# umutdundar99/progressive-stable-diffusion

Hardware: AMD Instinct MI355X
Metric: images/sec at 512x512, 50 DDIM steps, bs/GPU=4 (higher is better)
Workload: dtype f16; 1 GPU; 512x512, 50 DDIM steps, bs=4/GPU, delta-steer lambda=3.0, routing gates on, conditioning prep + VAE decode included; global_batch=4, parallelism=batch-shard x1 + 1 all-gather of uint8 frames

## Files before the change

### progressive-stable-diffusion_amd/csrc/bf16_names.h

```cpp
#pragma once
#define DADD_BF16 1

#define IgemmArgs IgemmArgs_bf16

#define igemm_kernel igemm_kernel_bf16
#define splitk_finish_kernel splitk_finish_kernel_bf16
#define splitk_finish_gn_kernel splitk_finish_gn_kernel_bf16
#define splitk_finish_gnapply_kernel splitk_finish_gnapply_kernel_bf16
#define igemm_dma_kernel igemm_dma_kernel_bf16
#define conv3x3_halo_kernel conv3x3_halo_kernel_bf16
#define gn_stats_kernel gn_stats_kernel_bf16
#define gn_apply_kernel gn_apply_kernel_bf16
#define gn_fused_kernel gn_fused_kernel_bf16
#define gn_reduce_kernel gn_reduce_kernel_bf16
#define layernorm_kernel layernorm_kernel_bf16
#define flash_kernel flash_kernel_bf16
#define xattn_kernel xattn_kernel_bf16
#define conv_in_nchw_kernel conv_in_nchw_kernel_bf16
#define conv_in_nchw_gn_kernel conv_in_nchw_gn_kernel_bf16
#define conv_cout4_kernel conv_cout4_kernel_bf16

#define dadd_init_igemm dadd_init_igemm_bf16
#define dadd_init_igemm_dma dadd_init_igemm_dma_bf16
#define dadd_launch_igemm_dma dadd_launch_igemm_dma_bf16
#define dadd_igemm_dma_persistent dadd_igemm_dma_persistent_bf16
#define dadd_init_conv_halo dadd_init_conv_halo_bf16
#define dadd_conv_halo_applicable dadd_conv_halo_applicable_bf16
#define dadd_conv_halo_gn_channels dadd_conv_halo_gn_channels_bf16
#define dadd_launch_conv_halo dadd_launch_conv_halo_bf16
#define dadd_init_norm dadd_init_norm_bf16
#define dadd_init_attention dadd_init_attention_bf16

#define dadd_conv_igemm_f16 dadd_conv_igemm_bf16
#define dadd_groupnorm_f16 dadd_groupnorm_bf16
#define dadd_layernorm_f16 dadd_layernorm_bf16
#define dadd_attn_f16 dadd_attn_bf16
#define dadd_attn_debug dadd_attn_debug_bf16
#define dadd_self_attn_f16 dadd_self_attn_bf16
#define dadd_tri_xattn_f16 dadd_tri_xattn_bf16
#define dadd_conv_in_nchw_f16 dadd_conv_in_nchw_bf16
#define dadd_conv3x3_cout4_f16 dadd_conv3x3_cout4_bf16
#define dadd_conv_out_ddim_f16 dadd_conv_out_ddim_bf16
```

### progressive-stable-diffusion_amd/csrc/igemm.hip

```cpp
#include "dadd_common.h"
#include "igemm_args.h"
#include <cstdlib>
#include <string>
#include "igemm_epilogue.h"

namespace {

constexpr int BM = 128;
constexpr int BK = 64;

__device__ __forceinline__ int lds_off(int row, int chunk) {
  return (row * 8 + (chunk ^ ((row >> 1) & 7))) * 8;
}

template <int BM, int BN, bool DEEP>
__global__ __launch_bounds__(256, 2) void igemm_kernel(const IgemmArgs p) {
  constexpr int WM = BM / 2;
  constexpr int MI = WM / 16;
  constexpr int WN = BN / 2;
  constexpr int J = WN / 16;
  constexpr int NA = BM * 8 / 256;
  constexpr int NB = BN * 8 / 256;
  extern __shared__ __attribute__((aligned(16))) char smem[];
  half_t* As = reinterpret_cast<half_t*>(smem);
// ... 512 lines not shown
  if (dma && tile_m == 128 && dadd_igemm_dma_persistent(a, nsplit) &&
      ((d->flags & DADD_TUNE_SHALLOW) ? false : 2.0 * a.B * a.Hi * a.Wi * Cin >= 2.0 * a.N * a.K))
    a.gm = a.gn = 0;
  const bool halo = dma && tile_m == 128 && dadd_conv_halo_applicable(a, tile_n);
  int halo_ns = 1;
  if (halo) {
    const int chunks = Cin / BK;
    int sk = d->splitk > 1 ? d->splitk : 1;
    if (sk > chunks) sk = chunks;
    a.kps = (chunks + sk - 1) / sk;
    halo_ns = (chunks + a.kps - 1) / a.kps;
    a.splitk = halo_ns;
    DADD_REQUIRE(halo_ns == 1 || a.partial != nullptr, "igemm: split-K needs a partial buffer");
  }
  if ((a.flags & DADD_EPI_GNSTAT) && (halo ? halo_ns : nsplit) > 1) {
    const int cb = (a.N % 160 == 0) ? 160 : 128, howo = a.Ho * a.Wo;
    const int rows = a.gn_nchunk > 0 ? howo / a.gn_nchunk : 0;
    DADD_REQUIRE(a.gn_ws && a.gn_cg > 0 && a.N == 32 * a.gn_cg && !geglu && a.counters == nullptr && a.N % cb == 0 &&
                     cb % a.gn_cg == 0 && (rows == 16 || rows == 64) && a.M % rows == 0 && howo % rows == 0 &&
                     a.gn_nchunk * rows == howo && !(a.flags & (DADD_EPI_LNFOLD | DADD_EPI_ACT_MASK)),
                 "igemm: GroupNorm statistics with split-K need the finish kernel (no tickets), N == 32 groups in blocks of "
                 "160 / 128 columns, and chunks of 16 or 64 rows: gn_nchunk == Ho*Wo / 16 (or / 64)");
  } else if (a.flags & DADD_EPI_GNSTAT) {
    const int wm_rows = tile_m / 2, wn_cols = tile_n / 2, howo = a.Ho * a.Wo;
    DADD_REQUIRE(a.gn_ws && a.gn_cg > 0 && a.N == 32 * a.gn_cg && !geglu && (tile_n == 128 || tile_n == 160) &&
                     wn_cols % a.gn_cg == 0 && a.M % tile_m == 0 && a.N % tile_n == 0 && howo % wm_rows == 0 &&
                     a.gn_nchunk == howo / wm_rows && !(a.flags & (DADD_EPI_LNFOLD | DADD_EPI_ACT_MASK)),
                 "igemm: GroupNorm statistics need full tiles of 128/160 columns holding whole groups, whole-wave row blocks "
                 "inside one sample (Ho*Wo %% %d == 0, gn_nchunk == Ho*Wo / %d), N == 32 groups, no split-K", wm_rows, wm_rows);
  }
  if (a.flags & DADD_EPI_GNAPPLY) {
    DADD_REQUIRE((halo ? halo_ns : nsplit) > 1 && a.counters == nullptr && a.gno_out && a.gno_gamma && a.gno_beta &&
                     a.gno_eps > 0.f && a.N % 64 == 0 && a.ldo % 2 == 0 && a.ldr % 2 == 0 &&
                     (size_t)a.Ho * a.Wo * (a.N / 32) * 2 <= 16 * 1024 && dadd_aligned16(a.gno_out) &&
                     !(a.flags & (DADD_EPI_GNSTAT | DADD_EPI_LNFOLD | DADD_EPI_LNSTAT | DADD_EPI_ACT_MASK)),
                 "igemm: GroupNorm of the output in the finish kernel needs a finish-kernel split-K launch, gn_out / gamma / "
                 "beta / eps, N %% 64 == 0, a (sample, group) slab of <= 16 KiB and no other statistics / activation flags");
  } else {
    DADD_REQUIRE(!(a.flags & DADD_EPI_GNAPPLY_SILU), "igemm: DADD_EPI_GNAPPLY_SILU without DADD_EPI_GNAPPLY");
  }
  if (a.flags & DADD_EPI_LNSTAT) {
    const int wn_cols = tile_n / 2;
    DADD_REQUIRE(a.ln_stats_out && !geglu && !halo && a.N % wn_cols == 0 && d->ln_parts_out == a.N / wn_cols &&
                     (nsplit == 1 || a.counters != nullptr) && !(a.flags & DADD_EPI_GNSTAT),
                 "igemm: LayerNorm row partials need ln_stats_out, N %% (tile_n/2) == 0, ln_parts_out == N / (tile_n/2) = %d, "
                 "no GEGLU and no finish-kernel split-K", a.N / wn_cols);
  }
  if (a.flags & DADD_PRE_GN) {
    const int cgc = Cin / 32;
    DADD_REQUIRE(a.C2 == 0 || (a.gni_ws2 && a.gni_nchunk2 >= 1 && a.gni_nchunk2 <= 256 && cgc > 0 && a.C1 % 32 == 0 &&
                               a.C2 % 32 == 0 && cgc % (a.C1 / 32) == 0 && cgc % (a.C2 / 32) == 0 && a.C1 % cgc == 0),
                 "igemm: GroupNorm over a concatenation needs the partials of both sources and group widths that nest "
                 "((C1+C2)/32 a multiple of C1/32 and C2/32, dividing C1)");
    DADD_REQUIRE(halo && !(d->flags & DADD_TUNE_SHALLOW) && Cin <= dadd_conv_halo_gn_channels(a.Wo) &&
                     Cin % 32 == 0 && a.gni_ws &&
                     a.gni_gamma && a.gni_beta && a.gni_nchunk >= 1 && a.gni_nchunk <= 256 && a.gni_eps > 0.f,
                 "igemm: GroupNorm on the way in needs the 3x3 halo kernel (stride 1, 64/32/16-wide map, 128x160 tiles), "
                 "Cin <= 1152 / 2048 / 2432 (W = 64 / 32 / 16), the chunk partials (<= 256 chunks), gamma, beta and eps");
  } else {
    DADD_REQUIRE(!(a.flags & DADD_PRE_GN_SILU), "igemm: DADD_PRE_GN_SILU without DADD_PRE_GN");
  }
  if (halo) {
    if (d->flags & DADD_TUNE_SHALLOW) a.flags |= DADD_TUNE_SHALLOW;
    rc = dadd_launch_conv_halo(a, halo_ns, s);
  }
  else if (dma)
    rc = dadd_launch_igemm_dma(a, tile_m, tile_n, nsplit, s);
  else if (tile_m == 128)
    rc = (tile_n == 160) ? launch<128, 160, false>(a, nsplit, s) : launch2<128, 128>(a, nsplit, deep, s);
  else
    rc = (tile_n == 160) ? launch2<64, 160>(a, nsplit, deep, s) : launch2<64, 128>(a, nsplit, deep, s);
  if (rc != DADD_OK) return rc;
  if ((halo ? halo_ns : nsplit) > 1 && a.counters == nullptr) {
    const size_t total = (size_t)a.M * (a.N / 4);
    int blocks = (int)((total + 255) / 256);
    if (blocks > 2048) blocks = 2048;
    const int ns = halo ? halo_ns : nsplit;
    const DaddLaunchTag tag = {(a.flags & DADD_EPI_GNSTAT) ? DADD_KNAME("splitk_finish_gn_kernel") : DADD_KNAME("splitk_finish_kernel"), 0.0,
                               (double)a.M * a.N * (4.0 * ns + 2.0 + ((a.flags & DADD_EPI_RESIDUAL) ? 2.0 : 0.0))};
    if (a.flags & DADD_EPI_GNAPPLY) {
      const DaddLaunchTag tag2 = {DADD_KNAME("splitk_finish_gnapply_kernel"), 0.0, tag.bytes + 2.0 * a.M * a.N};
      const unsigned slab_bytes = (unsigned)(a.Ho * a.Wo * (a.N / 32) * 2);
      if ((a.N / 32) % 4 == 0 && a.ldo % 4 == 0 && a.ldr % 4 == 0 && a.ld_rowvec % 4 == 0)
        dadd_launch(tag2, splitk_finish_gnapply_kernel<4>, dim3(32, a.B), dim3(512), slab_bytes, s, a, ns);
      else
        dadd_launch(tag2, splitk_finish_gnapply_kernel<2>, dim3(32, a.B), dim3(512), slab_bytes, s, a, ns);
    } else if (!(a.flags & DADD_EPI_GNSTAT))
      dadd_launch(tag, splitk_finish_kernel, dim3(blocks), dim3(256), 0, s, a, ns);
    else {
      const int rows = (a.Ho * a.Wo) / a.gn_nchunk;
      if (a.N % 160 == 0) {
        if (rows == 16) dadd_launch(tag, splitk_finish_gn_kernel<160, 16>, dim3(a.M / 16, a.N / 160), dim3(256), 0, s, a, ns);
        else dadd_launch(tag, splitk_finish_gn_kernel<160, 64>, dim3(a.M / 64, a.N / 160), dim3(256), 0, s, a, ns);
      } else {
        if (rows == 16) dadd_launch(tag, splitk_finish_gn_kernel<128, 16>, dim3(a.M / 16, a.N / 128), dim3(256), 0, s, a, ns);
        else dadd_launch(tag, splitk_finish_gn_kernel<128, 64>, dim3(a.M / 64, a.N / 128), dim3(256), 0, s, a, ns);
      }
    }
    DADD_LAUNCH_CHECK();
  }
  return DADD_OK;
}
```

### progressive-stable-diffusion_amd/csrc/igemm_args.h

```cpp
#pragma once
#include "dadd_common.h"

struct IgemmArgs {
  const half_t* x;
  const half_t* x2;
  const half_t* w;
  half_t* out;
  float* partial;
  const float* bias;
  const float* rowvec;
  const half_t* residual;
  int* counters;
  float* gn_ws;
  int gn_nchunk, gn_cg;
  const float* ln_c1;
  float ln_eps;
  float* ln_stats_out;
  const float* ln_stats_in;
  int ln_parts_in;
  const float* gni_ws;
  const float* gni_gamma;
  const float* gni_beta;
  int gni_nchunk;
  float gni_eps;
// ... 25 lines not shown
    const int per = p.gm * p.ntiles;
    const int g = tile_id / per, idx = tile_id - g * per;
    const int base = g * p.gm;
    const int gsz = min(p.gm, p.mtiles - base);
    mt = base + idx % gsz;
    nt = idx / gsz;
  } else if (p.gm >= p.mtiles) {
    const int per = p.mtiles * p.gn;
    const int g = tile_id / per, idx = tile_id - g * per;
    mt = idx % p.mtiles;
    nt = g * p.gn + idx / p.mtiles;
  } else {
    const int per = p.gm * p.gn;
    const int g = tile_id / per, idx = tile_id - g * per;
    const int ngn = p.ntiles / p.gn;
    const int gmi = g / ngn, gni = g - gmi * ngn;
    mt = gmi * p.gm + idx % p.gm;
    nt = gni * p.gn + idx / p.gm;
  }
}

static inline double dadd_igemm_flop(const IgemmArgs& a) { return 2.0 * (double)a.M * (double)a.N * (double)a.K; }
static inline double dadd_igemm_bytes(const IgemmArgs& a) {
  const double n_out = (a.flags & DADD_EPI_GEGLU) ? a.N / 2 : a.N;
  return 2.0 * ((double)a.B * a.Hi * a.Wi * (a.C1 + a.C2) + (double)a.N * a.K + (double)a.M * n_out +
                ((a.flags & DADD_EPI_RESIDUAL) ? (double)a.M * a.N : 0.0));
}

typedef half_t dadd_h2 __attribute__((ext_vector_type(2)));
__device__ __forceinline__ void ln_acc_pair(const h8& x, int p, float& s1, float& s2) {
  const dadd_h2 v = {x[2 * p], x[2 * p + 1]};
  const dadd_h2 one = {(half_t)1.0f, (half_t)1.0f};
  s1 = dadd_fdot2(v, one, s1);
  s2 = dadd_fdot2(v, v, s2);
}
template <int MI>
__device__ __forceinline__ void ln_finish(float (&s1)[MI], float (&s2)[MI], int K, float eps) {
  const float inv = 1.0f / (float)K;
#pragma unroll
  for (int i = 0; i < MI; ++i) {
    float a = s1[i], q = s2[i];
    a = dadd_sum_x16x32(a);
    q = dadd_sum_x16x32(q);
    const float mu = a * inv;
    const float var = fmaxf(q * inv - mu * mu, 0.f);
    s1[i] = mu;
    s2[i] = rsqrtf(var + eps);
  }
}

int dadd_init_igemm_dma();
int dadd_launch_igemm_dma(const IgemmArgs& a, int tile_m, int tile_n, int nsplit, hipStream_t s);
bool dadd_igemm_dma_persistent(const IgemmArgs& a, int nsplit);
int dadd_init_conv_halo();
bool dadd_conv_halo_applicable(const IgemmArgs& a, int tile_n);
int dadd_conv_halo_gn_channels(int Wo);
int dadd_launch_conv_halo(const IgemmArgs& a, int nsplit, hipStream_t s);
```

### progressive-stable-diffusion_amd/csrc/igemm_dma.hip

```cpp
#include "dadd_common.h"
#include "igemm_args.h"
#include <cstdlib>
#include "igemm_epilogue.h"

namespace {

constexpr int BK = 64;

typedef __attribute__((address_space(3))) void* lptr_t;
constexpr unsigned OOB = 0x80000000u;

__device__ __forceinline__ int lds_off(int row, int chunk) {
  return (row * 8 + (chunk ^ ((row >> 1) & 7))) * 8;
}

template <int N>
__device__ __forceinline__ void wait_vmcnt() {
  asm volatile("s_waitcnt vmcnt(%0)" ::"n"(N) : "memory");
}

template <int BM, int BN, bool UPS, bool PERS, int LNK>
__global__ __launch_bounds__(512, (BM + BN) <= 128 ? 4 : 2) void igemm_dma_kernel(const IgemmArgs p) {
#if defined(__HIP_DEVICE_COMPILE__)
  constexpr bool WS = true;
  constexpr bool LNF = LNK == 1;
  constexpr int WM = BM / 2, MI = WM / 16;
  constexpr int WN = BN / 2;
  constexpr int J = WN / 16;
  constexpr int NA = BM / 32;
  constexpr int NBJ = BN / 32;
  constexpr int LPT = NA + NBJ;
  constexpr int A_BYTES = BM * BK * 2, B_BYTES = BN * BK * 2, STAGE = A_BYTES + B_BYTES;
  extern __shared__ __attribute__((aligned(1024))) char smem[];

  const int t = threadIdx.x, lane = t & 63;
  const int wave_all = __builtin_amdgcn_readfirstlane(t >> 6);
  const bool loader = WS && wave_all >= 4;
  const int wave = WS ? (wave_all & 3) : wave_all;
  const int wm = wave >> 1, wn = wave & 1;
  int tile_first, tile_count;
  if constexpr (PERS) {
    const int total = p.mtiles * p.ntiles, nwg = gridDim.x;
    const int l = xcd_remap(blockIdx.x, nwg);
    const int q = total / nwg, r = total - q * nwg;
    tile_first = l * q + min(l, r);
    tile_count = q + (l < r ? 1 : 0);
  } else {
    tile_first = xcd_remap(blockIdx.x, gridDim.x);
    tile_count = 1;
  }
  const int z = PERS ? 0 : blockIdx.y;
  const int kt0 = PERS ? 0 : z * p.kps;
  const int kt1 = PERS ? p.nkt : min(p.nkt, kt0 + p.kps);
  const int nk = kt1 - kt0;
  const int Cin = p.C1 + p.C2;
  const int Hv = UPS ? 2 * p.Hi : p.Hi;
  const int Wv = UPS ? 2 * p.Wi : p.Wi;
  const int HoWo = p.Ho * p.Wo;
  const int lrow = lane >> 3, lch = lane & 7;

  const int shift1 = UPS ? 0 : (p.pad * p.Wi + p.pad) * p.C1;
  const int shift2 = UPS ? 0 : (p.pad * p.Wi + p.pad) * p.C2;
  const size_t pix_total = (size_t)p.B * p.Hi * p.Wi;
  const int rec1 = (int)((pix_total * p.C1 + shift1) * 2);
  const int rec2 = (int)((pix_total * p.C2 + shift2) * 2);
  const int recW = (int)((size_t)p.N * p.K * 2);
  const half_t* base1 = p.x - shift1;
  const half_t* base2 = (p.x2 ? p.x2 : p.x) - shift2;

  unsigned a_v1[NA], a_v2[NA], a_mask[NA];
  int a_pix[NA], a_y[NA], a_x[NA], a_cc[NA];
  unsigned w_v[NBJ];
  auto setup_tile = [&](int tile_id) {
  int nt, mt;
// ... 124 lines not shown
  const int total_kt = tile_count * nk;
  char* const ln_scr = smem + 4 * STAGE;
  const bool ln_stage = LNK == 2 && !UPS && ln_lds_usable(p, BM, nk);
  const bool ln_sts = ln_stage && ln_lds_stats(p, LN_LDS_BYTES);
  if (loader) {
    const int ln_extra = ln_stage ? ln_lds_count(p, wave, ln_sts) : 0;
    issue();
    issue();
    issue();
    wait_vmcnt<LPT>();
    __builtin_amdgcn_s_barrier();
    bool ext_young = false;
    int kc = 0, ext_tile = tile_first;
    for (int it = 0; it < total_kt; ++it) {
      if (it > 0) {
        if (ext_young) {
          switch (ln_extra) {
            case 1: wait_vmcnt<LPT + 1>(); break;
            case 2: wait_vmcnt<LPT + 2>(); break;
            case 3: wait_vmcnt<LPT + 3>(); break;
            case 4: wait_vmcnt<LPT + 4>(); break;
            default: wait_vmcnt<LPT>(); break;
          }
          ext_young = false;
        } else {
          wait_vmcnt<LPT>();
        }
        __builtin_amdgcn_s_barrier();
      }
      issue();
      if (ln_stage) {
        if (kc == 0) {
          int nt, mt;
          tile_decode(p, ext_tile, mt, nt);
          ln_lds_issue<BN>(p, ln_scr, __builtin_amdgcn_readfirstlane(mt) * BM, __builtin_amdgcn_readfirstlane(nt) * BN, wave,
                           lane, ln_sts);
          ext_young = ln_extra > 0;
          ++ext_tile;
        }
        kc = kc + 1 == nk ? 0 : kc + 1;
      }
    }
    wait_vmcnt<0>();
    return;
  }
  f4 acc[J][MI];
  const int fq = lane >> 4;
  int fa[2], fb[2];
#pragma unroll
  for (int s2 = 0; s2 < 2; ++s2) {
    fa[s2] = lds_off(wm * WM + (lane & 15), s2 * 4 + fq) * 2;
    fb[s2] = A_BYTES + lds_off(wn * WN + (lane & 15), s2 * 4 + fq) * 2;
  }
  __builtin_amdgcn_s_barrier();
  __builtin_amdgcn_sched_barrier(0);
  h8 xa0[MI], wb0[J], xa1[MI], wb1[J];
#pragma unroll
  for (int i = 0; i < MI; ++i) xa0[i] = *reinterpret_cast<const h8*>(smem + fa[0] + i * 2048);
#pragma unroll
  for (int j = 0; j < J; ++j) wb0[j] = *reinterpret_cast<const h8*>(smem + fb[0] + j * 2048);
  int comp_off = 0;
  bool started = false;
  for (int tl = 0; tl < tile_count; ++tl) {
#pragma unroll
    for (int j = 0; j < J; ++j)
#pragma unroll
      for (int i = 0; i < MI; ++i) acc[j][i] = f4{0.f, 0.f, 0.f, 0.f};
    [[maybe_unused]] float ls1[MI], ls2[MI];
    constexpr int LQ = MI * 4, LPER = (LQ + MI * J - 1) / (MI * J);
    if constexpr (LNF) {
#pragma unroll
      for (int i = 0; i < MI; ++i) ls1[i] = ls2[i] = 0.f;
    }
    for (int it = 0; it < nk; ++it) {
      if (started) __builtin_amdgcn_s_barrier();
      started = true;
      __builtin_amdgcn_sched_barrier(0);
      const int n1 = comp_off + STAGE;
      const int next_off = n1 >= 4 * STAGE ? 0 : n1;
      const char* ca = smem + comp_off + fa[1];
      const char* cb1 = smem + comp_off + fb[1];
      const char* na = smem + next_off + fa[0];
      const char* nb = smem + next_off + fb[0];
#pragma unroll
      for (int k = 0; k < MI * J; ++k) {
        const int jj = k / MI, ii = k % MI;
        acc[jj][ii] = DADD_MFMA_16X16X32(wb0[jj], xa0[ii], acc[jj][ii], 0, 0, 0);
        if constexpr (LNF) {
#pragma unroll
          for (int t2 = 0; t2 < LPER; ++t2)
            if (k * LPER + t2 < LQ) ln_acc_pair(xa0[(k * LPER + t2) / 4], (k * LPER + t2) % 4, ls1[(k * LPER + t2) / 4], ls2[(k * LPER + t2) / 4]);
        }
        if (k == 0) wb1[0] = *reinterpret_cast<const h8*>(cb1);
        else if (k <= MI) xa1[k - 1] = *reinterpret_cast<const h8*>(ca + (k - 1) * 2048);
        else if (k < MI + J) wb1[k - MI] = *reinterpret_cast<const h8*>(cb1 + (k - MI) * 2048);
        __builtin_amdgcn_sched_barrier(0);
      }
#pragma unroll
      for (int k = 0; k < MI * J; ++k) {
        const int jj = k / MI, ii = k % MI;
        acc[jj][ii] = DADD_MFMA_16X16X32(wb1[jj], xa1[ii], acc[jj][ii], 0, 0, 0);
        if constexpr (LNF) {
#pragma unroll
          for (int t2 = 0; t2 < LPER; ++t2)
            if (k * LPER + t2 < LQ) ln_acc_pair(xa1[(k * LPER + t2) / 4], (k * LPER + t2) % 4, ls1[(k * LPER + t2) / 4], ls2[(k * LPER + t2) / 4]);
        }
        if (k == 0) wb0[0] = *reinterpret_cast<const h8*>(nb);
        else if (k <= MI) xa0[k - 1] = *reinterpret_cast<const h8*>(na + (k - 1) * 2048);
        else if (k < MI + J) wb0[k - MI] = *reinterpret_cast<const h8*>(nb + (k - MI) * 2048);
        __builtin_amdgcn_sched_barrier(0);
      }
      comp_off = next_off;
      __builtin_amdgcn_sched_barrier(0);
    }
    int nt, mt;
    tile_decode(p, tile_first + tl, mt, nt);
    if constexpr (LNF) {
      ln_finish<MI>(ls1, ls2, p.K, p.ln_eps);
      igemm_epilogue<J, MI, WM, WN>(p, acc, mt * BM, nt * BN, wm, wn, lane, z, smem, ls1, ls2);
    } else {
      igemm_epilogue<J, MI, WM, WN>(p, acc, mt * BM, nt * BN, wm, wn, lane, z, smem, nullptr, nullptr, smem + 4 * STAGE,
                                    ln_sts ? ln_scr + LN_LDS_STATS : nullptr, ln_stage ? ln_scr : nullptr);
    }
  }
#endif
}

template <int BM, int BN>
constexpr int smem_bytes() {
  return 4 * (BM + BN) * BK * 2 + (BM == 128 ? LN_LDS_BYTES : 4096);
}

template <int BM, int BN, bool UPS, bool PERS, int LNK>
int set_attr() {
  DADD_HIP(hipFuncSetAttribute(reinterpret_cast<const void*>(&igemm_dma_kernel<BM, BN, UPS, PERS, LNK>),
                               hipFuncAttributeMaxDynamicSharedMemorySize, smem_bytes<BM, BN>()));
  return DADD_OK;
}

int g_num_cu = 0;

template <int BM, int BN, bool UPS, bool PERS, int LNK>
void launch1(const char* name, const IgemmArgs& a, dim3 grid, hipStream_t s) {
  dadd_launch({name, dadd_igemm_flop(a), dadd_igemm_bytes(a)}, igemm_dma_kernel<BM, BN, UPS, PERS, LNK>, grid, dim3(512),
              smem_bytes<BM, BN>(), s, a);
}
template <int BM, int BN, bool UPS, bool PERS>
void launch(const char* const (&names)[3], const IgemmArgs& a, dim3 grid, hipStream_t s) {
  if constexpr (!UPS) {
    if ((a.flags & DADD_EPI_LNFOLD) && a.ln_stats_in == nullptr) {
      launch1<BM, BN, false, PERS, 1>(names[1], a, grid, s);
      return;
    }
    if constexpr (BM == 128) {
      if (a.flags & DADD_EPI_LNFOLD) {
        launch1<BM, BN, false, PERS, 2>(names[2], a, grid, s);
        return;
      }
    }
  }
  launch1<BM, BN, UPS, PERS, 0>(names[0], a, grid, s);
}
template <int BM, int BN, bool PERS>
int set_attr2() {
  int rc = set_attr<BM, BN, false, PERS, 0>();
  if (rc == DADD_OK) rc = set_attr<BM, BN, false, PERS, 1>();
  if constexpr (BM == 128) {
    if (rc == DADD_OK) rc = set_attr<BM, BN, false, PERS, 2>();
  }
  return rc;
}

}

int dadd_init_igemm_dma() {
  int rc = set_attr2<128, 128, true>();
  if (rc == DADD_OK) rc = set_attr2<128, 160, true>();
  if (rc == DADD_OK) rc = set_attr2<128, 128, false>();
  if (rc == DADD_OK) rc = set_attr2<128, 160, false>();
  if (rc == DADD_OK) rc = set_attr<128, 128, true, false, 0>();
  if (rc == DADD_OK) rc = set_attr<128, 160, true, false, 0>();
  if (rc == DADD_OK) rc = set_attr2<64, 64, false>();
  if (rc == DADD_OK) rc = set_attr2<64, 128, false>();
  if (rc == DADD_OK) rc = set_attr2<64, 160, false>();
  int dev = 0;
  DADD_HIP(hipGetDevice(&dev));
  DADD_HIP(hipDeviceGetAttribute(&g_num_cu, hipDeviceAttributeMultiprocessorCount, dev));
  return rc;
}

bool dadd_igemm_dma_persistent(const IgemmArgs& a, int nsplit) {
  return (a.flags & DADD_TUNE_PERSIST) && nsplit == 1 && !a.ups && g_num_cu > 0 && a.mtiles * a.ntiles > g_num_cu;
}

int dadd_launch_igemm_dma(const IgemmArgs& a, int tile_m, int tile_n, int nsplit, hipStream_t s) {
  const int total = a.mtiles * a.ntiles;
  DADD_REQUIRE((size_t)a.B * a.Hi * a.Wi * (size_t)(a.C1 > a.C2 ? a.C1 : a.C2) * 2 < 0x7FF00000ull &&
                   (size_t)a.N * a.K * 2 < 0x7FF00000ull,
               "igemm(dma): operand larger than the 2 GiB buffer window");
  if (tile_m == 128 && dadd_igemm_dma_persistent(a, nsplit)) {
    dim3 grid(g_num_cu);
    if (tile_n == 160) { static const char* const nm[3] = {DADD_KNAME("igemm_dma_kernel") "<128, 160, false, true, 0>", DADD_KNAME("igemm_dma_kernel") "<128, 160, false, true, 1>", DADD_KNAME("igemm_dma_kernel") "<128, 160, false, true, 2>"}; launch<128, 160, false, true>(nm, a, grid, s); }
    else { static const char* const nm[3] = {DADD_KNAME("igemm_dma_kernel") "<128, 128, false, true, 0>", DADD_KNAME("igemm_dma_kernel") "<128, 128, false, true, 1>", DADD_KNAME("igemm_dma_kernel") "<128, 128, false, true, 2>"}; launch<128, 128, false, true>(nm, a, grid, s); }
    DADD_LAUNCH_CHECK();
    return DADD_OK;
  }
  dim3 grid(total, nsplit);
  if (tile_m == 64) {
    DADD_REQUIRE(!a.ups, "igemm(dma): the 64-row tiles have no upsample gather");
    if (tile_n == 160) { static const char* const nm[3] = {DADD_KNAME("igemm_dma_kernel") "<64, 160, false, false, 0>", DADD_KNAME("igemm_dma_kernel") "<64, 160, false, false, 1>", DADD_KNAME("igemm_dma_kernel") "<64, 160, false, false, 2>"}; launch<64, 160, false, false>(nm, a, grid, s); }
    else if (tile_n == 128) { static const char* const nm[3] = {DADD_KNAME("igemm_dma_kernel") "<64, 128, false, false, 0>", DADD_KNAME("igemm_dma_kernel") "<64, 128, false, false, 1>", DADD_KNAME("igemm_dma_kernel") "<64, 128, false, false, 2>"}; launch<64, 128, false, false>(nm, a, grid, s); }
    else { static const char* const nm[3] = {DADD_KNAME("igemm_dma_kernel") "<64, 64, false, false, 0>", DADD_KNAME("igemm_dma_kernel") "<64, 64, false, false, 1>", DADD_KNAME("igemm_dma_kernel") "<64, 64, false, false, 2>"}; launch<64, 64, false, false>(nm, a, grid, s); }
  } else if (tile_n == 160) {
    if (a.ups) { static const char* const nm[3] = {DADD_KNAME("igemm_dma_kernel") "<128, 160, true, false, 0>", DADD_KNAME("igemm_dma_kernel") "<128, 160, true, false, 1>", DADD_KNAME("igemm_dma_kernel") "<128, 160, true, false, 2>"}; launch<128, 160, true, false>(nm, a, grid, s); }
    else { static const char* const nm[3] = {DADD_KNAME("igemm_dma_kernel") "<128, 160, false, false, 0>", DADD_KNAME("igemm_dma_kernel") "<128, 160, false, false, 1>", DADD_KNAME("igemm_dma_kernel") "<128, 160, false, false, 2>"}; launch<128, 160, false, false>(nm, a, grid, s); }
  } else {
    if (a.ups) { static const char* const nm[3] = {DADD_KNAME("igemm_dma_kernel") "<128, 128, true, false, 0>", DADD_KNAME("igemm_dma_kernel") "<128, 128, true, false, 1>", DADD_KNAME("igemm_dma_kernel") "<128, 128, true, false, 2>"}; launch<128, 128, true, false>(nm, a, grid, s); }
    else { static const char* const nm[3] = {DADD_KNAME("igemm_dma_kernel") "<128, 128, false, false, 0>", DADD_KNAME("igemm_dma_kernel") "<128, 128, false, false, 1>", DADD_KNAME("igemm_dma_kernel") "<128, 128, false, false, 2>"}; launch<128, 128, false, false>(nm, a, grid, s); }
  }
  DADD_LAUNCH_CHECK();
  return DADD_OK;
}
```

### progressive-stable-diffusion_amd/engine.py

```python
from __future__ import annotations

import math
import os
from typing import Dict, List, Optional, Tuple

import torch

from . import lib as L
from .routing import get_block_type

F16, F32, BF16 = torch.float16, torch.float32, torch.bfloat16
OPERAND_DTYPES = (F16, BF16)
UNET_CH = (320, 640, 1280, 1280)
VAE_CH = (128, 256, 512, 512)
HEADS = 8
GROUPS = 32
N_CU = 256
FUSED_ATTN2 = os.environ.get("DADD_FUSED_ATTN2", "1") == "1"
A2_MIN_TILES = int(os.environ.get("DADD_A2_MIN_TILES", "128"))


def pack_conv(w: torch.Tensor, dtype=F16) -> torch.Tensor:
    if w.dim() == 2:
        return w.to(dtype).contiguous()
# ... 25 lines not shown

def fold_layernorm(w: torch.Tensor, b: Optional[torch.Tensor], gamma: torch.Tensor, beta: torch.Tensor, dtype=F16):
    w, gamma, beta = w.double(), gamma.double(), beta.double()
    w16 = (w * gamma[None, :]).to(dtype)
    bias = w @ beta + (b.double() if b is not None else 0.0)
    return w16, w16.double().sum(dim=1).float(), bias.float()


def lds_image(w: torch.Tensor) -> torch.Tensor:
    r = w.shape[0]
    sw = (torch.arange(r) >> 1) & 7
    idx = (torch.arange(8)[None, :] ^ sw[:, None])
    return w.reshape(r, 8, 8).gather(1, idx[:, :, None].expand(r, 8, 8)).reshape(r, 64).contiguous()


def pack_ffn_stream(w1: torch.Tensor, b1: torch.Tensor, w2: torch.Tensor, wp: torch.Tensor):
    c, hid = 320, 1280
    assert tuple(w1.shape) == (2 * hid, c) and tuple(w2.shape) == (c, hid) and tuple(wp.shape)[:2] == (c, c)
    w1, w2, wp = w1.to(F16), w2.to(F16), wp.reshape(c, c).to(F16)
    pieces, bias = [], []
    e = torch.arange(16)
    for ch in range(hid // 64):
        rows = []
        for wn in range(2):
            for u in range(2):
                h = ch * 64 + wn * 32 + u * 16 + e
                rows += [h, hid + h]
                bias += [b1[h].float(), b1[hid + h].float()]
        rows = torch.cat(rows)
        for kt in range(c // 64):
            pieces.append(lds_image(w1[rows][:, kt * 64:(kt + 1) * 64]))
        for nh in range(2):
            pieces.append(lds_image(w2[nh * 160:(nh + 1) * 160, ch * 64:(ch + 1) * 64]))
    for nh in range(2):
        for kt in range(c // 64):
            pieces.append(lds_image(wp[nh * 160:(nh + 1) * 160, kt * 64:(kt + 1) * 64]))
    return torch.cat([p.reshape(-1) for p in pieces]).contiguous(), torch.cat(bias).contiguous()


def pack_head_stream(wp: torch.Tensor, wq: torch.Tensor, wk: torch.Tensor, wv: torch.Tensor) -> torch.Tensor:
    c = 320
    wp = wp.reshape(c, c).to(F16)
    wqkv = torch.cat([wq, wk, wv]).to(F16)
    assert tuple(wqkv.shape) == (3 * c, c)
    pieces = []
    for w in (wp, wqkv):
        for nh in range(w.shape[0] // 160):
            for kt in range(c // 64):
                pieces.append(lds_image(w[nh * 160:(nh + 1) * 160, kt * 64:(kt + 1) * 64]))
    return torch.cat([p.reshape(-1) for p in pieces]).contiguous()


GN_IN_CONV = True

HALO_DUO = False

FINISH_GN_APPLY = True

WEIGHT_PREFETCH_AHEAD = int(os.environ.get("DADD_WEIGHT_PREFETCH", "0"))
WEIGHT_PREFETCH_MIN_BYTES = 2 * 1024 * 1024

GN_FROM_EPILOGUE = True
GN_FUSED_MAX_BYTES = 16 * 1024
SPLITK_GN_ROWS = 16


LN_FOLD = "auto"
LN_STATS_FROM_PRODUCER = True
LN_STATS_MAX_PARTS = 8


FUSED_FFN = True
FFN_MIN_BLOCKS = 128
FUSED_HEAD = True


def fold_here(m: int, n: int, k: int, geglu: bool = False) -> bool:
    if LN_FOLD == "auto":
        tile_m, _, _, tune = plan_tiling(m, n, k, 1, geglu, False)
        return tile_m == 64 and not (tune & L.TUNE_NODMA)
    return bool(LN_FOLD)


def choose_tiling(m: int, n: int, k: int, tile_n: int, geglu: bool = False,
                  residual: bool = True) -> Tuple[int, int, int]:
    nkt = k // 64
    nt = math.ceil(n / tile_n)
    t128 = math.ceil(m / 128) * nt
    if geglu:
        if m >= 16384:
            return 64, 1, L.TUNE_NODMA | L.TUNE_SHALLOW
        return 128, 1, (L.TUNE_PERSIST if t128 >= 4 * N_CU else 0)
    if nkt >= 12:
        if n <= 128 and nkt <= 18:
            return 128, 1, L.TUNE_NODMA
        per = 16 if t128 > 64 else (10 if t128 > 16 else 8)
        sk = max(1, min(round(N_CU / t128), nkt // per, 32))
        if not residual and nkt <= 20:
            sk = 1
        return 128, sk, (L.TUNE_PERSIST if sk == 1 and t128 >= 8 * N_CU else 0)
    if t128 > N_CU:
        return 128, 1, L.TUNE_PERSIST
    if not residual and nkt >= 5:
        return 128, 1, 0
    return (128 if t128 >= 2 * N_CU else 64), 1, L.TUNE_NODMA

# ... 133 lines not shown
                ws = self.be.zeros((out_shape[0] * (nchunk + extra) * GROUPS * 2,), F32)
                self.keep.append(ws)
                self.gn_partials[out.data_ptr()] = (ws, nchunk)
                gkw = dict(gn_ws=ws, gn_nchunk=nchunk)
                flags |= L.EPI_GNSTAT
        if (ln_stats and LN_STATS_FROM_PRODUCER and not (flags & (L.EPI_GEGLU | L.EPI_GNSTAT)) and sk == 1
                and n % (tile_n // 2) == 0 and n // (tile_n // 2) <= LN_STATS_MAX_PARTS):
            st = self.be.zeros((n // (tile_n // 2), m, 2), F32)
            self.keep.append(st)
            self.ln_partials[out.data_ptr()] = st
            gkw["ln_stats_out"] = st
            flags |= L.EPI_LNSTAT
        f = flags | (L.EPI_BIAS if bias is not None else 0) | (L.EPI_ROWVEC if rowvec is not None else 0) \
            | (L.EPI_RESIDUAL if residual is not None else 0) | (L.EPI_LNFOLD if ln_c1 is not None else 0) | tune
        kw = dict(ln_c1=ln_c1, ln_eps=ln_eps) if ln_c1 is not None else {}
        if (fuse_gn is not None and FINISH_GN_APPLY and sk > 1 and self.sk_counters is None and not (f & L.EPI_GNSTAT)
                and n % 64 == 0 and out_shape[1] * out_shape[2] * (n // 32) * 2 <= GN_FUSED_MAX_BYTES):
            g_out = self.pool.get(out_shape)
            f |= L.EPI_GNAPPLY | (L.EPI_GNAPPLY_SILU if fuse_gn[3] else 0)
            kw["gn_apply"] = (g_out, fuse_gn[0], fuse_gn[1], fuse_gn[2])
            self.gn_ready[out.data_ptr()] = (g_out, fuse_gn[0].data_ptr(), fuse_gn[1].data_ptr(), float(fuse_gn[2]), bool(fuse_gn[3]))
        if gn_in is not None:
            f |= L.PRE_GN | (L.PRE_GN_SILU if gn_in[5] else 0)
            kw["gn_in"] = tuple(gn_in[:5]) + tuple(gn_in[6:])
        if ln_c1 is not None and ln_stats_in is not None:
            kw["ln_stats_in"] = ln_stats_in
        self.rec(self.be.igemm, x, w, out, x2=x2, bias=bias, rowvec=rowvec, residual=residual,
                 taps=taps, stride=stride, ups=ups, pad=pad, flags=f, splitk=sk, partial=partial,
                 tile_n=tile_n, tile_m=tile_m, counters=self.sk_counters if sk > 1 else None, **kw, **gkw)
        self.pool.put(partial)
        return out

    def gn_in_conv_ok(self, x, x2, w, out_shape, residual) -> Optional[Tuple]:
        cmax = {64: 1152, 32: 2048, 16: 2432}.get(x.shape[2], 0)
        cin = x.shape[-1] + (0 if x2 is None else x2.shape[-1])
        if not GN_IN_CONV or cin > cmax or x.shape[-1] % 64 or cin % 64:
            return None
        part = self.gn_partials.get(x.data_ptr())
        if part is None or part[1] > 128:
            return None
        if x2 is not None:
            part2 = self.gn_partials.get(x2.data_ptr())
            c1_, c2_, cgc = x.shape[-1], x2.shape[-1], cin // 32
            if (part2 is None or part2[1] > 128 or c1_ % 32 or c2_ % 32 or cgc % (c1_ // 32) or cgc % (c2_ // 32)
                    or c1_ % cgc):
                return None
            part = (part[0], part[1], part2[0], part2[1])
        b, h, w_, _ = x.shape
        n, m = w.shape[0], out_shape[0] * out_shape[1] * out_shape[2]
        if tuple(out_shape[1:3]) != (h, w_) or h != w_ or w_ not in (16, 32, 64) or (h * w_) % 128:
            return None
        tile_m, tile_n, _, tune = plan_tiling(m, n, w.shape[1], 9, False, residual is not None, 0, 1)
        if tile_m != 128 or tile_n != 160 or (tune & (L.TUNE_NODMA | L.TUNE_PERSIST)) or HALO_DUO:
            return None
        return part

    def gn(self, x1, x2, gamma, beta, eps, silu):
        c = x1.shape[-1] + (0 if x2 is None else x2.shape[-1])
        ready = self.gn_ready.get(x1.data_ptr()) if x2 is None else None
        if ready is not None and ready[1:] == (gamma.data_ptr(), beta.data_ptr(), float(eps), bool(silu)):
            del self.gn_ready[x1.data_ptr()]
            return ready[0]
        out = self.pool.get((*x1.shape[:3], c))
        part = self.gn_partials.get(x1.data_ptr()) if x2 is None else None
        if part is not None:
            self.rec(self.be.groupnorm, x1, None, gamma, beta, out, part[0], GROUPS, eps, silu, ws_chunks=part[1])
        else:
            self.rec(self.be.groupnorm, x1, x2, gamma, beta, out, self.gn_ws, GROUPS, eps, silu)
        return out


class UNetPlan(_Plan):

    def __init__(self, be, sd: Dict[str, torch.Tensor], batch: int, side: int, *,
                 prefix="unet.unet", use_routing_gates=True, use_frequency_strategy=True, wcache=None, dtype=F16):
        super().__init__(be, wcache, dtype)
        assert side % 8 == 0, "latent side must be a multiple of 8 (three stride-2 levels)"
        self.B, self.S = batch, side
        self.gates_mode = use_routing_gates
        self.prefix = prefix + "."
        self.sd = sd
        self.lam = 0.0
        self.params = be.zeros((2,), F32)
        self.params_dev = False
        self.ddim_coef = None
        self.gn_ws = be.empty((batch * L.GN_MAX_CHUNKS * GROUPS * 2,), F32)
        u = self.prefix
        self.w_t1 = self.dev(sd[u + "time_embedding.linear_1.weight"], F16)
        self.b_t1 = self.dev(sd[u + "time_embedding.linear_1.bias"])
        self.w_t2 = self.dev(sd[u + "time_embedding.linear_2.weight"], F16)
        self.b_t2 = self.dev(sd[u + "time_embedding.linear_2.bias"])
        names = self._resnet_names()
        self.temb_off, off = {}, 0
        for nme in names:
            self.temb_off[nme] = off
            off += sd[u + nme + ".time_emb_proj.weight"].shape[0]
        self.temb_cols = off
        self.w_tp = self.dev(torch.cat([sd[u + n + ".time_emb_proj.weight"] for n in names]), F16)
        self.b_tp = self.dev(torch.cat([sd[u + n + ".time_emb_proj.bias"] for n in names]))
        self.temb_rows = be.zeros((batch, self.temb_cols), F32)
        self.sites = self._attn_sites()
        self.T = 48 if use_routing_gates else 32
        self.kv_w, self.kv, self.gates = {}, {}, {}
        for site, c in self.sites:
            ap = f"{u}{site}.transformer_blocks.0.attn2"
            ws = [sd[ap + ".to_k.weight"], sd[ap + ".to_v.weight"]]
# ... 115 lines not shown
        else:
            g2 = self.gn(h1, None, self.f(name + ".norm2.weight"), self.f(name + ".norm2.bias"), 1e-5, 1)
            self.pool.put(h1)
            out = self.conv(g2, w2, (b, h, w_, cout), bias=self.f(name + ".conv2.bias"), residual=res, gn_stats=True, fuse_gn=next_gn)
            self.pool.put(g2)
        if res is not x:
            self.pool.put(res)
        return out

    def _ln_linear(self, tb, norm, name, wkey_list, bias_key=None, geglu=False):
        u = self.prefix

        def make():
            w = torch.cat([self.sd[u + tb + k] for k in wkey_list])
            b = self.sd[u + tb + bias_key] if bias_key else None
            w16, c1, bias = fold_layernorm(w, b, self.sd[u + tb + norm + ".weight"], self.sd[u + tb + norm + ".bias"],
                                           self.dtype)
            if geglu:
                idx = geglu_interleave(torch.arange(w16.shape[0])[:, None].float(), torch.zeros(w16.shape[0]))[0][:, 0].long()
                w16, c1, bias = w16[idx], c1[idx], bias[idx]
            return self.dev(w16.contiguous()), self.dev(c1.contiguous()), self.dev(bias.contiguous())
        t = self.cached((u + tb, "lnfold", name), make)
        if self.wcache is not None:
            self.keep += list(t)
        return t

    def _transformer(self, site, x):
        b, h, w_, c = x.shape
        shp = (b, h, w_, c)
        tb = site + ".transformer_blocks.0"
        m_rows = b * h * w_
        fold1, fold2, fold3 = (fold_here(m_rows, 3 * c, c), fold_here(m_rows, c, c) and site not in self.a2,
                               fold_here(m_rows, 8 * c, c, True))
        rowblock = self.dtype == F16
        fused_tail = rowblock and FUSED_FFN and c == 320 and (h * w_) % 64 == 0 and m_rows // 64 >= FFN_MIN_BLOCKS
        xpart = self.gn_partials.get(x.data_ptr())
        fused_head = (rowblock and FUSED_HEAD and c == 320 and (h * w_) % 64 == 0 and m_rows // 64 >= FFN_MIN_BLOCKS
                      and xpart is not None and xpart[1] <= 256)
        ext = LN_STATS_FROM_PRODUCER and LN_FOLD == "auto"
        if fused_head:
            u = self.prefix

            def _head():
                return self.dev(pack_head_stream(self.sd[u + site + ".proj_in.weight"], *[self.sd[u + tb + f".attn1.to_{n}.weight"] for n in "qkv"]))
            hstream = self.cached((self.prefix + tb, "head_stream"), _head)
            if self.wcache is not None:
                self.keep.append(hstream)
            hs = self.pool.get(shp)
            qkv = self.pool.get((b, h, w_, 3 * c))
            self.rec(self.be.tf_head, x.view(b, h * w_, c), hstream, xpart[0], xpart[1], self.f(site + ".norm.weight"),
                     self.f(site + ".norm.bias"), self.f(site + ".proj_in.bias"), self.f(tb + ".norm1.weight"),
                     self.f(tb + ".norm1.bias"), hs.view(b, h * w_, c), qkv.view(b, h * w_, 3 * c))
        else:
            g = self.gn(x, None, self.f(site + ".norm.weight"), self.f(site + ".norm.bias"), 1e-6, 0)
            hs = self.conv(g, self.w(site + ".proj_in.weight"), shp, bias=self.f(site + ".proj_in.bias"),
                           taps=1, pad=0, ln_stats=LN_STATS_FROM_PRODUCER and LN_FOLD == "auto" and not fold1)
            self.pool.put(g)
        ln_box = [None]

        def ln_of(src, norm):
            if ln_box[0] is None:
                ln_box[0] = self.pool.get(shp)
            self.rec(self.be.layernorm, src, self.f(tb + norm + ".weight"), self.f(tb + norm + ".bias"), ln_box[0])
            return ln_box[0]
        st1 = self.ln_partials.get(hs.data_ptr())
        if fused_head:
            pass
        elif fold1 or st1 is not None:
            wqkv, c1, bqkv = self._ln_linear(tb, ".norm1", "qkv", [f".attn1.to_{n}.weight" for n in "qkv"])
            qkv = self.conv(hs, wqkv, (b, h, w_, 3 * c), bias=bqkv, taps=1, pad=0, ln_c1=c1,
                            ln_stats_in=None if fold1 else st1)
        else:
            wqkv = self.cached((self.prefix + tb, "qkv"), lambda: self.dev(
                torch.cat([self.sd[self.prefix + tb + f".attn1.to_{n}.weight"] for n in "qkv"]), self.dtype))
            qkv = self.conv(ln_of(hs, ".norm1"), wqkv, (b, h, w_, 3 * c), taps=1, pad=0)
        att = self.pool.get(shp)
        self.rec(self.be.self_attn, qkv.view(b, h * w_, 3 * c), att.view(b, h * w_, c), HEADS)
        self.pool.put(qkv)
        fused2 = site in self.a2
        h2 = self.conv(att, self.w(tb + ".attn1.to_out.0.weight"), shp,
                       bias=self.f(tb + ".attn1.to_out.0.bias"), residual=hs, taps=1, pad=0,
                       ln_stats=ext and not fold2)
        self.pool.put(hs)
        st3 = None
        if fused2:
            st = self.a2[site]
            st2 = self.ln_partials.get(h2.data_ptr())
            kw2 = {}
            if st2 is not None:
                st["fold"] = True
                lnx = h2
                kw2 = dict(ln_stats_in=st2, ln_c1=st["ln_c1"], ln_d=st["ln_d"], ln_eps=1e-5)
            else:
                lnx = ln_of(h2, ".norm2")
            h3 = self.pool.get(shp)
            if ext and not fold3 and c % 80 == 0 and not fused_tail:
                st3 = self.be.zeros((c // 80, m_rows, 2), F32)
                self.keep.append(st3)
                kw2["ln_stats_out"] = st3
            self.rec(self.be.attn2_fused, lnx.view(b, h * w_, c), st["mcat"], st["vw"],
                     self.f(tb + ".attn2.to_out.0.bias"), h2.view(b, h * w_, c), h3.view(b, h * w_, c), **kw2)
        else:
            st2 = self.ln_partials.get(h2.data_ptr())
            if fold2 or st2 is not None:
                wq, c1, bq = self._ln_linear(tb, ".norm2", "to_q", [".attn2.to_q.weight"])
                q = self.conv(h2, wq, shp, bias=bq, taps=1, pad=0, ln_c1=c1, ln_stats_in=None if fold2 else st2)
            else:
                q = self.conv(ln_of(h2, ".norm2"), self.w(tb + ".attn2.to_q.weight"), shp, taps=1, pad=0)
            self.rec(self._xattn, site, q.view(b, h * w_, c), att.view(b, h * w_, c))
            self.pool.put(q)
# ... 474 lines not shown
```

Before: 10.67 images/sec.

## Fuse GroupNorm into the 1x1 proj_in linear on LDS-DMA 64-row tiles

Adds a GNI variant of the LDS-DMA igemm kernel. Each workgroup reduces the GroupNorm chunk partials for its sample, builds a per-channel scale/shift table in LDS, and applies it to the A fragments before the MFMA loop. The transformer proj_in path uses this when the tiling and partials allow, so it skips a separate GroupNorm kernel and the write and re-read of the normalized activation. In exchange it adds per-workgroup statistic reduction in double precision, extra LDS that can lower occupancy, and ALU work in the inner loop.

```diff
diff --git a/progressive-stable-diffusion_amd/csrc/bf16_names.h b/progressive-stable-diffusion_amd/csrc/bf16_names.h
--- a/progressive-stable-diffusion_amd/csrc/bf16_names.h
+++ b/progressive-stable-diffusion_amd/csrc/bf16_names.h
@@ -24,6 +24,7 @@
 #define dadd_init_igemm_dma dadd_init_igemm_dma_bf16
 #define dadd_launch_igemm_dma dadd_launch_igemm_dma_bf16
 #define dadd_igemm_dma_persistent dadd_igemm_dma_persistent_bf16
+#define dadd_igemm_dma_gn_channels dadd_igemm_dma_gn_channels_bf16
 #define dadd_init_conv_halo dadd_init_conv_halo_bf16
 #define dadd_conv_halo_applicable dadd_conv_halo_applicable_bf16
 #define dadd_conv_halo_gn_channels dadd_conv_halo_gn_channels_bf16
diff --git a/progressive-stable-diffusion_amd/csrc/igemm.hip b/progressive-stable-diffusion_amd/csrc/igemm.hip
--- a/progressive-stable-diffusion_amd/csrc/igemm.hip
+++ b/progressive-stable-diffusion_amd/csrc/igemm.hip
@@ -588,11 +588,16 @@
                                a.C2 % 32 == 0 && cgc % (a.C1 / 32) == 0 && cgc % (a.C2 / 32) == 0 && a.C1 % cgc == 0),
                  "igemm: GroupNorm over a concatenation needs the partials of both sources and group widths that nest "
                  "((C1+C2)/32 a multiple of C1/32 and C2/32, dividing C1)");
-    DADD_REQUIRE(halo && !(d->flags & DADD_TUNE_SHALLOW) && Cin <= dadd_conv_halo_gn_channels(a.Wo) &&
-                     Cin % 32 == 0 && a.gni_ws &&
-                     a.gni_gamma && a.gni_beta && a.gni_nchunk >= 1 && a.gni_nchunk <= 256 && a.gni_eps > 0.f,
-                 "igemm: GroupNorm on the way in needs the 3x3 halo kernel (stride 1, 64/32/16-wide map, 128x160 tiles), "
-                 "Cin <= 1152 / 2048 / 2432 (W = 64 / 32 / 16), the chunk partials (<= 256 chunks), gamma, beta and eps");
+    DADD_REQUIRE(Cin % 32 == 0 && a.gni_ws && a.gni_gamma && a.gni_beta && a.gni_nchunk >= 1 && a.gni_nchunk <= 256 &&
+                     a.gni_eps > 0.f,
+                 "igemm: GroupNorm on the way in needs the chunk partials (<= 256 chunks), gamma, beta and eps");
+    const bool gni = dma && !halo && tile_m == 64 && a.taps == 1 && a.pad == 0 && a.stride == 1 && !a.ups && a.C2 == 0 &&
+                     nsplit == 1 && (a.Ho * a.Wo) % 64 == 0 && Cin <= dadd_igemm_dma_gn_channels(tile_n) &&
+                     !(a.flags & (DADD_PRE_GN_SILU | DADD_EPI_LNFOLD));
+    DADD_REQUIRE(gni || (halo && !(d->flags & DADD_TUNE_SHALLOW) && Cin <= dadd_conv_halo_gn_channels(a.Wo)),
+                 "igemm: GroupNorm on the way in needs the 3x3 halo kernel (stride 1, 64/32/16-wide map, 128x160 tiles, "
+                 "Cin <= 1152 / 2048 / 2432 at W = 64 / 32 / 16) or a 1x1 linear on 64-row LDS-DMA tiles (one source, "
+                 "Ho*Wo %% 64 == 0, no SiLU, no folded LayerNorm, no split-K, Cin <= %d)", dadd_igemm_dma_gn_channels(tile_n));
   } else {
     DADD_REQUIRE(!(a.flags & DADD_PRE_GN_SILU), "igemm: DADD_PRE_GN_SILU without DADD_PRE_GN");
   }
diff --git a/progressive-stable-diffusion_amd/csrc/igemm_args.h b/progressive-stable-diffusion_amd/csrc/igemm_args.h
--- a/progressive-stable-diffusion_amd/csrc/igemm_args.h
+++ b/progressive-stable-diffusion_amd/csrc/igemm_args.h
@@ -101,6 +101,7 @@
 int dadd_init_igemm_dma();
 int dadd_launch_igemm_dma(const IgemmArgs& a, int tile_m, int tile_n, int nsplit, hipStream_t s);
 bool dadd_igemm_dma_persistent(const IgemmArgs& a, int nsplit);
+int dadd_igemm_dma_gn_channels(int tile_n);
 int dadd_init_conv_halo();
 bool dadd_conv_halo_applicable(const IgemmArgs& a, int tile_n);
 int dadd_conv_halo_gn_channels(int Wo);
diff --git a/progressive-stable-diffusion_amd/csrc/igemm_dma.hip b/progressive-stable-diffusion_amd/csrc/igemm_dma.hip
--- a/progressive-stable-diffusion_amd/csrc/igemm_dma.hip
+++ b/progressive-stable-diffusion_amd/csrc/igemm_dma.hip
@@ -19,7 +19,25 @@
   asm volatile("s_waitcnt vmcnt(%0)" ::"n"(N) : "memory");
 }
 
-template <int BM, int BN, bool UPS, bool PERS, int LNK>
+template <int BM, int BN>
+constexpr int smem_bytes() {
+  return 4 * (BM + BN) * BK * 2 + (BM == 128 ? LN_LDS_BYTES : 4096);
+}
+constexpr int LDS_LIMIT = 160 * 1024;
+
+__device__ __forceinline__ void gn_frag(h8& v, const f4 (&t)[4]) {
+  const float sc[8] = {t[0][0], t[0][2], t[1][0], t[1][2], t[2][0], t[2][2], t[3][0], t[3][2]};
+  const float sh[8] = {t[0][1], t[0][3], t[1][1], t[1][3], t[2][1], t[2][3], t[3][1], t[3][3]};
+#pragma unroll
+  for (int e = 0; e < 8; ++e) v[e] = (half_t)((float)v[e] * sc[e] + sh[e]);
+}
+__device__ __forceinline__ void gn_pairs(f4 (&t)[4], const char* tab, int ch0) {
+  const f4* tb = reinterpret_cast<const f4*>(tab + ch0 * 8);
+#pragma unroll
+  for (int u = 0; u < 4; ++u) t[u] = tb[u];
+}
+
+template <int BM, int BN, bool UPS, bool PERS, int LNK, bool GNI = false>
 __global__ __launch_bounds__(512, (BM + BN) <= 128 ? 4 : 2) void igemm_dma_kernel(const IgemmArgs p) {
 #if defined(__HIP_DEVICE_COMPILE__)
   constexpr bool WS = true;
@@ -250,6 +268,48 @@
     fa[s2] = lds_off(wm * WM + (lane & 15), s2 * 4 + fq) * 2;
     fb[s2] = A_BYTES + lds_off(wn * WN + (lane & 15), s2 * 4 + fq) * 2;
   }
+  [[maybe_unused]] const char* const gtab = smem + smem_bytes<BM, BN>();
+  if constexpr (GNI) {
+    static_assert(!PERS && !UPS && LNK == 0, "GroupNorm on the A fragments: one 1x1 tile per workgroup, no LayerNorm fold");
+    int mt0, nt0;
+    tile_decode(p, tile_first, mt0, nt0);
+    const int b = (mt0 * BM) / HoWo;
+    const int cg = Cin >> 5;
+    const int g = wave * 8 + (lane >> 3), sub = lane & 7;
+    const int nch = p.gni_nchunk;
+    double a = 0.0, q = 0.0;
+    for (int k = sub; k < nch; k += 32) {
+      dadd_f2 v[4];
+#pragma unroll
+      for (int u = 0; u < 4; ++u) {
+        const int kk = min(k + 8 * u, nch - 1);
+        v[u] = *reinterpret_cast<const dadd_f2*>(p.gni_ws + (((size_t)b * nch + kk) * 32 + g) * 2);
+      }
+#pragma unroll
+      for (int u = 0; u < 4; ++u) {
+        if (k + 8 * u < nch) {
+          a += (double)v[u][0];
+          q += (double)v[u][1];
+        }
+      }
+    }
+#pragma unroll
+    for (int o = 4; o > 0; o >>= 1) {
+      a += __shfl_xor(a, o, 64);
+      q += __shfl_xor(q, o, 64);
+    }
+    const double n = (double)HoWo * (double)cg;
+    const double mu = a / n;
+    double var = q / n - mu * mu;
+    if (var < 0.0) var = 0.0;
+    const float mean_f = (float)mu, rstd_f = (float)(1.0 / sqrt(var + (double)p.gni_eps));
+    for (int cc = sub; cc < cg; cc += 8) {
+      const int ch = g * cg + cc;
+      const float sc = rstd_f * p.gni_gamma[ch];
+      *reinterpret_cast<dadd_f2*>(smem + smem_bytes<BM, BN>() + ch * 8) = dadd_f2{sc, p.gni_beta[ch] - mean_f * sc};
+    }
+    asm volatile("s_waitcnt lgkmcnt(0)" ::: "memory");
+  }
   __builtin_amdgcn_s_barrier();
   __builtin_amdgcn_sched_barrier(0);
   h8 xa0[MI], wb0[J], xa1[MI], wb1[J];
@@ -257,6 +317,9 @@
   for (int i = 0; i < MI; ++i) xa0[i] = *reinterpret_cast<const h8*>(smem + fa[0] + i * 2048);
 #pragma unroll
   for (int j = 0; j < J; ++j) wb0[j] = *reinterpret_cast<const h8*>(smem + fb[0] + j * 2048);
+  [[maybe_unused]] int gc = kt0 * BK;
+  [[maybe_unused]] f4 gt0[4], gt1[4];
+  if constexpr (GNI) gn_pairs(gt0, gtab, gc + fq * 8);
   int comp_off = 0;
   bool started = false;
   for (int tl = 0; tl < tile_count; ++tl) {
@@ -280,6 +343,12 @@
       const char* cb1 = smem + comp_off + fb[1];
       const char* na = smem + next_off + fa[0];
       const char* nb = smem + next_off + fb[0];
+      if constexpr (GNI) {
+#pragma unroll
+        for (int i = 0; i < MI; ++i) gn_frag(xa0[i], gt0);
+        gn_pairs(gt1, gtab, gc + (4 + fq) * 8);
+        __builtin_amdgcn_sched_barrier(0);
+      }
 #pragma unroll
       for (int k = 0; k < MI * J; ++k) {
         const int jj = k / MI, ii = k % MI;
@@ -292,6 +361,13 @@
         if (k == 0) wb1[0] = *reinterpret_cast<const h8*>(cb1);
         else if (k <= MI) xa1[k - 1] = *reinterpret_cast<const h8*>(ca + (k - 1) * 2048);
         else if (k < MI + J) wb1[k - MI] = *reinterpret_cast<const h8*>(cb1 + (k - MI) * 2048);
+        __builtin_amdgcn_sched_barrier(0);
+      }
+      if constexpr (GNI) {
+#pragma unroll
+        for (int i = 0; i < MI; ++i) gn_frag(xa1[i], gt1);
+        gc = gc + BK < Cin ? gc + BK : 0;
+        gn_pairs(gt0, gtab, gc + fq * 8);
         __builtin_amdgcn_sched_barrier(0);
       }
 #pragma unroll
@@ -324,11 +400,6 @@
 #endif
 }
 
-template <int BM, int BN>
-constexpr int smem_bytes() {
-  return 4 * (BM + BN) * BK * 2 + (BM == 128 ? LN_LDS_BYTES : 4096);
-}
-
 template <int BM, int BN, bool UPS, bool PERS, int LNK>
 int set_attr() {
   DADD_HIP(hipFuncSetAttribute(reinterpret_cast<const void*>(&igemm_dma_kernel<BM, BN, UPS, PERS, LNK>),
@@ -359,6 +430,18 @@
   }
   launch1<BM, BN, UPS, PERS, 0>(names[0], a, grid, s);
 }
+template <int BN>
+int set_attr_gni() {
+  DADD_HIP(hipFuncSetAttribute(reinterpret_cast<const void*>(&igemm_dma_kernel<64, BN, false, false, 0, true>),
+                               hipFuncAttributeMaxDynamicSharedMemorySize, LDS_LIMIT));
+  return DADD_OK;
+}
+template <int BN>
+void launch_gni(const char* name, const IgemmArgs& a, dim3 grid, hipStream_t s) {
+  dadd_launch({name, dadd_igemm_flop(a), dadd_igemm_bytes(a)}, igemm_dma_kernel<64, BN, false, false, 0, true>, grid, dim3(512),
+              smem_bytes<64, BN>() + (a.C1 + a.C2) * 8, s, a);
+}
+
 template <int BM, int BN, bool PERS>
 int set_attr2() {
   int rc = set_attr<BM, BN, false, PERS, 0>();
@@ -381,6 +464,9 @@
   if (rc == DADD_OK) rc = set_attr2<64, 64, false>();
   if (rc == DADD_OK) rc = set_attr2<64, 128, false>();
   if (rc == DADD_OK) rc = set_attr2<64, 160, false>();
+  if (rc == DADD_OK) rc = set_attr_gni<64>();
+  if (rc == DADD_OK) rc = set_attr_gni<128>();
+  if (rc == DADD_OK) rc = set_attr_gni<160>();
   int dev = 0;
   DADD_HIP(hipGetDevice(&dev));
   DADD_HIP(hipDeviceGetAttribute(&g_num_cu, hipDeviceAttributeMultiprocessorCount, dev));
@@ -389,6 +475,11 @@
 
 bool dadd_igemm_dma_persistent(const IgemmArgs& a, int nsplit) {
   return (a.flags & DADD_TUNE_PERSIST) && nsplit == 1 && !a.ups && g_num_cu > 0 && a.mtiles * a.ntiles > g_num_cu;
+}
+
+int dadd_igemm_dma_gn_channels(int tile_n) {
+  const int ring = tile_n == 160 ? smem_bytes<64, 160>() : (tile_n == 128 ? smem_bytes<64, 128>() : smem_bytes<64, 64>());
+  return (LDS_LIMIT - ring) / 8;
 }
 
 int dadd_launch_igemm_dma(const IgemmArgs& a, int tile_m, int tile_n, int nsplit, hipStream_t s) {
@@ -404,6 +495,15 @@
     return DADD_OK;
   }
   dim3 grid(total, nsplit);
+  if (a.flags & DADD_PRE_GN) {
+    DADD_REQUIRE(tile_m == 64 && !a.ups && a.C1 + a.C2 <= dadd_igemm_dma_gn_channels(tile_n),
+                 "igemm(dma): GroupNorm on the way in needs 64-row tiles and <= %d input channels", dadd_igemm_dma_gn_channels(tile_n));
+    if (tile_n == 160) launch_gni<160>(DADD_KNAME("igemm_dma_kernel") "<64, 160, false, false, 0, true>", a, grid, s);
+    else if (tile_n == 128) launch_gni<128>(DADD_KNAME("igemm_dma_kernel") "<64, 128, false, false, 0, true>", a, grid, s);
+    else launch_gni<64>(DADD_KNAME("igemm_dma_kernel") "<64, 64, false, false, 0, true>", a, grid, s);
+    DADD_LAUNCH_CHECK();
+    return DADD_OK;
+  }
   if (tile_m == 64) {
     DADD_REQUIRE(!a.ups, "igemm(dma): the 64-row tiles have no upsample gather");
     if (tile_n == 160) { static const char* const nm[3] = {DADD_KNAME("igemm_dma_kernel") "<64, 160, false, false, 0>", DADD_KNAME("igemm_dma_kernel") "<64, 160, false, false, 1>", DADD_KNAME("igemm_dma_kernel") "<64, 160, false, false, 2>"}; launch<64, 160, false, false>(nm, a, grid, s); }
diff --git a/progressive-stable-diffusion_amd/engine.py b/progressive-stable-diffusion_amd/engine.py
--- a/progressive-stable-diffusion_amd/engine.py
+++ b/progressive-stable-diffusion_amd/engine.py
@@ -101,6 +101,9 @@
 
 
 GN_IN_CONV = True
+
+GN_IN_LINEAR = True
+GN_IN_LINEAR_MIN_ROWS = 1024
 
 HALO_DUO = False
 
@@ -340,6 +343,21 @@
             return None
         tile_m, tile_n, _, tune = plan_tiling(m, n, w.shape[1], 9, False, residual is not None, 0, 1)
         if tile_m != 128 or tile_n != 160 or (tune & (L.TUNE_NODMA | L.TUNE_PERSIST)) or HALO_DUO:
+            return None
+        return part
+
+    def gn_in_linear_ok(self, x, w, out_shape) -> Optional[Tuple]:
+        b, h, w_, c = x.shape
+        m, n = b * h * w_, w.shape[0]
+        if (not GN_IN_LINEAR or m < GN_IN_LINEAR_MIN_ROWS or (h * w_) % 64 or c % 64 or w.shape[1] != c
+                or tuple(out_shape[:3]) != (b, h, w_) or x.data_ptr() in self.gn_ready):
+            return None
+        part = self.gn_partials.get(x.data_ptr())
+        if part is None or part[1] > 256:
+            return None
+        tile_m, tile_n, sk, tune = plan_tiling(m, n, c, 1, False, False)
+        ring = 4 * (64 + tile_n) * 64 * 2 + 4096
+        if tile_m != 64 or sk != 1 or (tune & L.TUNE_NODMA) or ring + 8 * c > 160 * 1024:
             return None
         return part
 
@@ -561,10 +579,17 @@
                      self.f(site + ".norm.bias"), self.f(site + ".proj_in.bias"), self.f(tb + ".norm1.weight"),
                      self.f(tb + ".norm1.bias"), hs.view(b, h * w_, c), qkv.view(b, h * w_, 3 * c))
         else:
-            g = self.gn(x, None, self.f(site + ".norm.weight"), self.f(site + ".norm.bias"), 1e-6, 0)
-            hs = self.conv(g, self.w(site + ".proj_in.weight"), shp, bias=self.f(site + ".proj_in.bias"),
-                           taps=1, pad=0, ln_stats=LN_STATS_FROM_PRODUCER and LN_FOLD == "auto" and not fold1)
-            self.pool.put(g)
+            w_in = self.w(site + ".proj_in.weight")
+            pin = self.gn_in_linear_ok(x, w_in, shp)
+            if pin is not None:
+                hs = self.conv(x, w_in, shp, bias=self.f(site + ".proj_in.bias"), taps=1, pad=0,
+                               ln_stats=LN_STATS_FROM_PRODUCER and LN_FOLD == "auto" and not fold1,
+                               gn_in=(pin[0], pin[1], self.f(site + ".norm.weight"), self.f(site + ".norm.bias"), 1e-6, 0))
+            else:
+                g = self.gn(x, None, self.f(site + ".norm.weight"), self.f(site + ".norm.bias"), 1e-6, 0)
+                hs = self.conv(g, w_in, shp, bias=self.f(site + ".proj_in.bias"),
+                               taps=1, pad=0, ln_stats=LN_STATS_FROM_PRODUCER and LN_FOLD == "auto" and not fold1)
+                self.pool.put(g)
         ln_box = [None]
 
         def ln_of(src, norm):
```

Result: no change. 10.75 images/sec (median of 6 runs) (+0.7%).
